# lkp411/cDLRM

Hardware: AMD Instinct MI355X
Metric: training samples/sec, Criteo-Terabyte-shape synthetic (cached data-parallel DLRM step; look-ahead refills that fall into the timed region included: see config.refills_in_timed_region) (higher is better)
Workload: dtype f32

## Files before the change

cdlrm_amd/csrc/dense.hip:

```cpp
#include "gemm_wide.h"
#include "gemm_bf16.h"

#define SK_KMAX 32
__global__ void __launch_bounds__(256) k_linear_smallk(const float* __restrict__ X, int64_t ld_x, const float* __restrict__ W,
                                                       const float* __restrict__ bias, float* __restrict__ Y, int64_t ld_y,
                                                       int64_t M, int N, int K, int act) {
    __shared__ float Xs[32][SK_KMAX + 1];
    __shared__ __attribute__((aligned(16))) float Wt[SK_KMAX][128 + 4];
    const int64_t m0 = (int64_t)blockIdx.y * 32;
    const int n0 = blockIdx.x * 128;
    for (int e = threadIdx.x; e < 32 * K; e += 256) {
        const int r = e / K, k = e % K;
        Xs[r][k] = X[min(m0 + r, M - 1) * ld_x + k];
    }
    for (int e = threadIdx.x; e < 128 * K; e += 256) {
        const int n = e / K, k = e % K;
        Wt[k][n] = W[(int64_t)min(n0 + n, N - 1) * K + k];
    }
    __syncthreads();
    const int cg = threadIdx.x & 31, rg = threadIdx.x >> 5;
    float acc[4][4];
#pragma unroll
    for (int i = 0; i < 4; ++i)
#pragma unroll
// ... 851 lines not shown
        const int off = itself ? 1 : 0;
#if IA_ABL == 3
        if (acc00[0] + acc10[1] + acc11[2] == 1.2345f) out[0] = 1.f;
#else
        for (int c = lane; c < D; c += 64) out[c] = Ts[c];
#pragma unroll
        for (int r = 0; r < 4; ++r) {
            const int i0 = 4 * g4 + r, i1 = 16 + 4 * g4 + r;
            if (i0 < F && l16 < i0 + off) out[D + pair_base(i0, itself) + l16] = acc00[r];
            if (i1 < F) out[D + pair_base(i1, itself) + l16] = acc10[r];
            if (i1 < F && 16 + l16 < i1 + off) out[D + pair_base(i1, itself) + 16 + l16] = acc11[r];
        }
#endif
        __builtin_amdgcn_sched_barrier(0);
        IA_STAMP_AT(3)
    };
    for (; b < B; b += nw) one(b);
}

struct IaGather {
    const TableDesc* tab;
    const v4f* weight;
    const int32_t* slots;
    int64_t n;
    int64_t ldx4;
    const uint8_t* once;
    int64_t ld_once;
    float lr;
};

template <int D4, int NS, bool G, bool DB = false>
__global__ void __launch_bounds__(256) k_interact_fwd_s(const float* __restrict__ feat, IaGather ga, int64_t B, int F,
                                                        int itself, float* __restrict__ R, int64_t ld_r) {
    constexpr int D = 4 * D4, CS = D4 / NS, DS = 4 * CS, PITCH = DS + 4, NR = CS / 2;
    constexpr int TSW = ia_fwd_s_slices(D4, NS, DB);
    static_assert(32 * PITCH == ia_slab_slice(D4, NS), "the slice the kernel walks is the slice the launch is sized for");
    static_assert(!DB || (NS % 2 == 0 && DS / 16 >= 1), "double buffering alternates two slices over an even number of slabs");
    extern __shared__ __attribute__((aligned(16))) float smem[];
    const int lane = threadIdx.x & 63, wave = threadIdx.x >> 6;
    float* Ts = smem + wave * ia_fwd_s_floats(D4, NS, DB);
    float* Os = Ts + TSW;
    const int64_t nw = (int64_t)gridDim.x * 4;
    int64_t b = (int64_t)blockIdx.x * 4 + wave;
    if (b >= B) return;
    const int l16 = lane & 15, g4 = lane >> 4;
    const int off = itself ? 1 : 0;
    int soff[NR], doff[NR];
    int srow[G ? NR : 1];
    const v4f* wbase[G ? NR : 1];
#pragma unroll
    for (int i = 0; i < NR; ++i) {
        const int e = lane + 64 * i, row = e / CS, c = e % CS;
        soff[i] = G ? c : min(row, F - 1) * D4 + c;
        doff[i] = row * PITCH + 4 * c;
        if constexpr (G) {
            const int t = max(min(row, F - 1) - 1, 0);
            srow[i] = t * (int)ga.n;
            wbase[i] = ga.weight + (ga.tab[t].row_base * D4 + c);
        }
    }
    v4f nxt[NS][NR];
    const v4f* pn[G ? NR : 1];
    int32_t sl[G ? NR : 1];
    auto load_slots = [&](int64_t bb) __attribute__((always_inline)) {
#pragma unroll
        for (int i = 0; i < NR; ++i) sl[i] = ga.slots[srow[i] + bb];
    };
    auto make_ptrs = [&](int64_t bb) __attribute__((always_inline)) {
#pragma unroll
        for (int i = 0; i < NR; ++i) {
            const v4f* p = wbase[i] + (int64_t)sl[i] * D4;
            if (i == 0 && lane < CS) p = reinterpret_cast<const v4f*>(feat) + bb * ga.ldx4 + soff[i];
            pn[i] = p;
        }
    };
    auto prefetch = [&](int s, int64_t bb) __attribute__((always_inline)) {
        if constexpr (G) {
#pragma unroll
            for (int i = 0; i < NR; ++i) nxt[s][i] = pn[i][s * CS];
        } else {
            const v4f* src = reinterpret_cast<const v4f*>(feat) + bb * (int64_t)F * D4 + s * CS;
#pragma unroll
            for (int i = 0; i < NR; ++i) nxt[s][i] = src[soff[i]];
        }
    };
    if constexpr (G) {
        load_slots(b);
        make_ptrs(b);
    }
#pragma unroll
    for (int s = 0; s < NS; ++s) prefetch(s, b);
    if constexpr (G) load_slots(min(b + nw, B - 1));
    if constexpr (DB) {
        float* const T0 = Ts;
        float* const T1 = Ts + 32 * PITCH;
        constexpr int NG = DS / 16;
#pragma unroll
        for (int i = 0; i < NR; ++i) *reinterpret_cast<v4f*>(T0 + doff[i]) = nxt[0][i];
        const int toff = l16 * PITCH + 4 * g4;
        float4 fa0 = *reinterpret_cast<const float4*>(T0 + toff);
        float4 fa1 = *reinterpret_cast<const float4*>(T0 + toff + 16 * PITCH);
        auto one_db = [&](int64_t b) __attribute__((always_inline)) {
            const int64_t bn = min(b + nw, B - 1);
            if constexpr (G) {
                make_ptrs(bn);
                load_slots(min(bn + nw, B - 1));
            }
            prefetch(0, bn);
            if (lane < CS) *reinterpret_cast<v4f*>(Os + 4 * lane) = *reinterpret_cast<const v4f*>(T0 + 4 * lane);
            v4f acc00 = {0.f, 0.f, 0.f, 0.f}, acc10 = acc00, acc11 = acc00;
            auto mf = [&](int j, const float4& a0, const float4& a1) __attribute__((always_inline)) {
                const int c = j / 3, w = j % 3;
                const float x0 = c == 0 ? a0.x : c == 1 ? a0.y : c == 2 ? a0.z : a0.w;
                const float x1 = c == 0 ? a1.x : c == 1 ? a1.y : c == 2 ? a1.z : a1.w;
                if (w == 0) acc00 = __builtin_amdgcn_mfma_f32_16x16x4f32(x0, x0, acc00, 0, 0, 0);
                else if (w == 1) acc10 = __builtin_amdgcn_mfma_f32_16x16x4f32(x1, x0, acc10, 0, 0, 0);
                else acc11 = __builtin_amdgcn_mfma_f32_16x16x4f32(x1, x1, acc11, 0, 0, 0);
            };
#pragma unroll
            for (int s = 0; s < NS; ++s) {
                const float* cur = (s & 1) ? T1 : T0;
                float* oth = (s & 1) ? T0 : T1;
#pragma unroll
                for (int g = 0; g < NG; ++g) {
                    const float4 a0 = fa0, a1 = fa1;
                    const float* np_ = (g + 1 < NG) ? cur + toff + 16 * (g + 1) : oth + toff;
#pragma unroll
                    for (int j = 0; j < 12; ++j) {
                        mf(j, a0, a1);
                        const int k = g * 12 + j;
                        if (k >= 0 && k < NR) {
                            const int sn = s + 1 < NS ? s + 1 : 0;
                            *reinterpret_cast<v4f*>(oth + doff[k]) = nxt[sn][k];
                        }
                        if (k == NR && s + 1 < NS && lane < CS) *reinterpret_cast<v4f*>(Os + (s + 1) * DS + 4 * lane) = nxt[s + 1][0];
                        if (k == NR + 1 && s + 1 < NS) prefetch(s + 1, bn);
                        if (j == (NG == 1 ? NR + 2 : 0) && g == NG - 1) {
                            fa0 = *reinterpret_cast<const float4*>(np_);
                            fa1 = *reinterpret_cast<const float4*>(np_ + 16 * PITCH);
                        }
                        if (j == 0 && g + 1 < NG) {
                            fa0 = *reinterpret_cast<const float4*>(np_);
                            fa1 = *reinterpret_cast<const float4*>(np_ + 16 * PITCH);
                        }
                        __builtin_amdgcn_sched_barrier(0);
                    }
                }
            }
            float* out = R + b * ld_r;
#pragma unroll
            for (int r = 0; r < 4; ++r) {
                const int i0 = 4 * g4 + r, i1 = 16 + 4 * g4 + r;
                if (i0 < F && l16 < i0 + off) Os[D + pair_base(i0, itself) + l16] = acc00[r];
                if (i1 < F) Os[D + pair_base(i1, itself) + l16] = acc10[r];
                if (i1 < F && 16 + l16 < i1 + off) Os[D + pair_base(i1, itself) + 16 + l16] = acc11[r];
            }
            const int width = D + pair_base(F, itself);
            if (lane < 4) Os[width + lane] = 0.f;
            const int W4 = (width + 3) >> 2;
            constexpr int NST = (D4 + 132 + 63) / 64;
#pragma unroll
            for (int k = 0; k < NST; ++k) {
                const int e = min(64 * k + lane, W4 - 1);
                *reinterpret_cast<v4f*>(out + 4 * e) = *reinterpret_cast<const v4f*>(Os + 4 * e);
            }
            __builtin_amdgcn_sched_barrier(0);
        };
        one_db(b);
        for (b += nw; b < B; b += nw) one_db(b);
        return;
    }
    auto one = [&](int64_t b) __attribute__((always_inline)) {
        const int64_t bn = min(b + nw, B - 1);
        if constexpr (G) {
            make_ptrs(bn);
            load_slots(min(bn + nw, B - 1));
        }
        v4f acc00 = {0.f, 0.f, 0.f, 0.f}, acc10 = acc00, acc11 = acc00;
        const float* tp = Ts + l16 * PITCH + 4 * g4;
#pragma unroll
        for (int s = 0; s < NS; ++s) {
#pragma unroll
            for (int i = 0; i < NR; ++i) *reinterpret_cast<v4f*>(Ts + doff[i]) = nxt[s][i];
            if (lane < CS) *reinterpret_cast<v4f*>(Os + s * DS + 4 * lane) = nxt[s][0];
            prefetch(s, bn);
            __builtin_amdgcn_sched_barrier(0);
#pragma unroll 2
            for (int g = 0; g < DS / 16; ++g) {
                const float4 a0 = *reinterpret_cast<const float4*>(tp + 16 * g);
                const float4 a1 = *reinterpret_cast<const float4*>(tp + 16 * PITCH + 16 * g);
                acc00 = __builtin_amdgcn_mfma_f32_16x16x4f32(a0.x, a0.x, acc00, 0, 0, 0);
                acc10 = __builtin_amdgcn_mfma_f32_16x16x4f32(a1.x, a0.x, acc10, 0, 0, 0);
                acc11 = __builtin_amdgcn_mfma_f32_16x16x4f32(a1.x, a1.x, acc11, 0, 0, 0);
                acc00 = __builtin_amdgcn_mfma_f32_16x16x4f32(a0.y, a0.y, acc00, 0, 0, 0);
                acc10 = __builtin_amdgcn_mfma_f32_16x16x4f32(a1.y, a0.y, acc10, 0, 0, 0);
                acc11 = __builtin_amdgcn_mfma_f32_16x16x4f32(a1.y, a1.y, acc11, 0, 0, 0);
                acc00 = __builtin_amdgcn_mfma_f32_16x16x4f32(a0.z, a0.z, acc00, 0, 0, 0);
                acc10 = __builtin_amdgcn_mfma_f32_16x16x4f32(a1.z, a0.z, acc10, 0, 0, 0);
                acc11 = __builtin_amdgcn_mfma_f32_16x16x4f32(a1.z, a1.z, acc11, 0, 0, 0);
                acc00 = __builtin_amdgcn_mfma_f32_16x16x4f32(a0.w, a0.w, acc00, 0, 0, 0);
                acc10 = __builtin_amdgcn_mfma_f32_16x16x4f32(a1.w, a0.w, acc10, 0, 0, 0);
                acc11 = __builtin_amdgcn_mfma_f32_16x16x4f32(a1.w, a1.w, acc11, 0, 0, 0);
            }
            __builtin_amdgcn_sched_barrier(0);
        }
        float* out = R + b * ld_r;
#pragma unroll
        for (int r = 0; r < 4; ++r) {
            const int i0 = 4 * g4 + r, i1 = 16 + 4 * g4 + r;
            if (i0 < F && l16 < i0 + off) Os[D + pair_base(i0, itself) + l16] = acc00[r];
            if (i1 < F) Os[D + pair_base(i1, itself) + l16] = acc10[r];
            if (i1 < F && 16 + l16 < i1 + off) Os[D + pair_base(i1, itself) + 16 + l16] = acc11[r];
        }
        const int width = D + pair_base(F, itself);
        if (lane < 4) Os[width + lane] = 0.f;
        const int W4 = (width + 3) >> 2;
        constexpr int NST = (D4 + 132 + 63) / 64;
#pragma unroll
        for (int k = 0; k < NST; ++k) {
            const int e = min(64 * k + lane, W4 - 1);
            *reinterpret_cast<v4f*>(out + 4 * e) = *reinterpret_cast<const v4f*>(Os + 4 * e);
        }
        __builtin_amdgcn_sched_barrier(0);
    };
    one(b);
    for (b += nw; b < B; b += nw) one(b);
}

template <int D4>
__global__ void __launch_bounds__(256) k_interact_bwd_p(const float* __restrict__ feat, const float* __restrict__ dR,
                                                        int64_t ld_r, int64_t B, int F, int itself, int x_act,
                                                        float* __restrict__ dfeat) {
    constexpr int D = 4 * D4, PITCH = D + 4;
    constexpr int GMAX = ia_grad_row(D4);
    constexpr int NG = (GMAX / 4 + 63) / 64;
    static_assert(32 * PITCH == ia_row_tile(D4), "the tile the kernel walks is the tile the launch is sized for");
    extern __shared__ __attribute__((aligned(16))) float smem[];
    const int lane = threadIdx.x & 63, wave = threadIdx.x >> 6;
    const int lr = lane & 31, lk = lane >> 5;
    float* Ts = smem + wave * ia_bwd_p_floats(D4);
    float* Gs = Ts + 32 * PITCH;
    for (int e = lane; e < 32 * PITCH; e += 64) Ts[e] = 0.f;
    const int FD4 = F * D4;
    const int off = itself ? 1 : 0;
    const int npairs = pair_base(F, itself);
    const int G4 = (D + npairs + 3) / 4;
    const int64_t nw = (int64_t)gridDim.x * 4;
    int64_t b = (int64_t)blockIdx.x * 4 + wave;
    if (b >= B) return;
    v4f nxt[D4 / 2], gn[NG];
    interact_prefetch<D4>(feat, b, FD4, lane, nxt);
#pragma unroll
    for (int i = 0; i < NG; ++i) gn[i] = reinterpret_cast<const v4f*>(dR + b * ld_r)[min(lane + 64 * i, G4 - 1)];
    auto one = [&](int64_t b) __attribute__((always_inline)) {
        interact_stage<D4>(Ts, FD4, lane, nxt);
#pragma unroll
        for (int i = 0; i < NG; ++i) *reinterpret_cast<v4f*>(Gs + 4 * min(lane + 64 * i, GMAX / 4 - 1)) = gn[i];
        const int64_t bn = min(b + nw, B - 1);
        interact_prefetch<D4>(feat, bn, FD4, lane, nxt);
#pragma unroll
        for (int i = 0; i < NG; ++i) gn[i] = reinterpret_cast<const v4f*>(dR + bn * ld_r)[min(lane + 64 * i, G4 - 1)];
        __builtin_amdgcn_sched_barrier(0);
        float sreg[16];
#pragma unroll
        for (int m = 0; m < 16; ++m) {
            const int j = lk + 2 * m;
            float v = 0.f;
            if (lr < F && j < F) {
                if (j < lr + off) v += Gs[D + pair_base(lr, itself) + j];
                if (lr < j + off) v += Gs[D + pair_base(j, itself) + lr];
            }
            sreg[m] = v;
        }
        float* out = dfeat + b * F * D;
        for (int n0 = 0; n0 < D; n0 += 32) {
            f32x16 acc;
#pragma unroll
            for (int r = 0; r < 16; ++r) acc[r] = 0.f;
            const float* tp = Ts + lk * PITCH + n0 + lr;
#pragma unroll
            for (int m = 0; m < 16; ++m) acc = __builtin_amdgcn_mfma_f32_32x32x2f32(sreg[m], tp[2 * m * PITCH], acc, 0, 0, 0);
            const int col = n0 + lr;
#pragma unroll
            for (int r = 0; r < 16; ++r) {
                const int i = (r & 3) + 8 * (r >> 2) + 4 * lk;
                if (i < F) {
                    float v = acc[r];
                    if (i == 0) {
                        v += Gs[col];
                        const float y = Ts[col];
                        if (x_act == 1) v = y > 0.f ? v : 0.f;
                        else if (x_act == 2) v = v * ((1.0f - y) * y);
                    }
                    out[i * D + col] = v;
                }
            }
        }
        __builtin_amdgcn_sched_barrier(0);
    };
    for (; b < B; b += nw) one(b);
}

template <int D4, int NS, bool G, bool ONCE = false>
__global__ void __launch_bounds__(256, (G && D4 <= 32) ? 2 : 1) k_interact_bwd_s(const float* __restrict__ feat, IaGather ga,
                                                        const float* __restrict__ dR, int64_t ld_r, int64_t B, int F,
                                                        int itself, int x_act, float* __restrict__ dfeat) {
    constexpr int D = 4 * D4, CS = D4 / NS, DS = 4 * CS, PITCH = DS + 4, NR = CS / 2;
    constexpr int GMAX = ia_grad_row(D4);
    constexpr int NG = (GMAX / 4 + 63) / 64;
    static_assert(DS % 32 == 0, "a slab is a whole number of 32-column MFMA blocks");
    static_assert(32 * PITCH == ia_slab_slice(D4, NS), "the slice the kernel walks is the slice the launch is sized for");
    extern __shared__ __attribute__((aligned(16))) float smem[];
    const int lane = threadIdx.x & 63, wave = threadIdx.x >> 6;
    const int lr = lane & 31, lk = lane >> 5;
    float* Ts = smem + wave * ia_bwd_s_floats(D4, NS);
    float* Gs = Ts + 32 * PITCH;
    float* Os = Gs + D;
    const int off = itself ? 1 : 0;
    const int npairs = pair_base(F, itself);
    const int G4 = (D + npairs + 3) / 4;
    const int64_t nw = (int64_t)gridDim.x * 4;
    int64_t b = (int64_t)blockIdx.x * 4 + wave;
    if (b >= B) return;
    int soff[NR], doff[NR];
    int srow[G ? NR : 1];
    int orow[ONCE ? NR : 1];
    const v4f* wbase[G ? NR : 1];
#pragma unroll
    for (int i = 0; i < NR; ++i) {
        const int e = lane + 64 * i, row = e / CS, c = e % CS;
        soff[i] = G ? c : min(row, F - 1) * D4 + c;
        doff[i] = row * PITCH + 4 * c;
        if constexpr (G) {
            const int t = max(min(row, F - 1) - 1, 0);
            srow[i] = t * (int)ga.n;
            if constexpr (ONCE) orow[i] = t * (int)ga.ld_once;
            wbase[i] = ga.weight + (ga.tab[t].row_base * D4 + c);
        }
    }
    static_assert(!ONCE || (G && CS == 8 && DS == 32), "the output store's lane -> (row, word) map is the staging map");
    v4f nxt[NS][NR], gn[NG];
    const v4f* pn[G ? NR : 1];
    int32_t sl[G ? NR : 1];
    const v4f* pc[ONCE ? NR : 1];
    uint8_t fl[ONCE ? NR : 1], fn[ONCE ? NR : 1], fc[ONCE ? NR : 1];
    auto load_slots = [&](int64_t bb) __attribute__((always_inline)) {
#pragma unroll
        for (int i = 0; i < NR; ++i) {
            sl[i] = ga.slots[srow[i] + bb];
            if constexpr (ONCE) fl[i] = ga.once[orow[i] + bb];
        }
    };
    auto make_ptrs = [&](int64_t bb) __attribute__((always_inline)) {
#pragma unroll
        for (int i = 0; i < NR; ++i) {
            const v4f* p = wbase[i] + (int64_t)sl[i] * D4;
            if constexpr (ONCE) fn[i] = fl[i];
            if (i == 0 && lane < CS) {
                p = reinterpret_cast<const v4f*>(feat) + bb * ga.ldx4 + soff[i];
                if constexpr (ONCE) fn[i] = 0;
            }
            pn[i] = p;
        }
    };
    auto prefetch = [&](int s, int64_t bb) __attribute__((always_inline)) {
        if constexpr (G) {
#pragma unroll
            for (int i = 0; i < NR; ++i) nxt[s][i] = pn[i][s * CS];
        } else {
            const v4f* src = reinterpret_cast<const v4f*>(feat) + bb * (int64_t)F * D4 + s * CS;
#pragma unroll
            for (int i = 0; i < NR; ++i) nxt[s][i] = src[soff[i]];
        }
    };
    if constexpr (G) {
        load_slots(b);
        make_ptrs(b);
    }
#pragma unroll
    for (int i = 0; i < NG; ++i) gn[i] = reinterpret_cast<const v4f*>(dR + b * ld_r)[min(lane + 64 * i, G4 - 1)];
#pragma unroll
    for (int s = 0; s < NS; ++s) prefetch(s, b);
    if constexpr (G) load_slots(min(b + nw, B - 1));
    auto one = [&](int64_t b) __attribute__((always_inline)) {
        const int64_t bn = min(b + nw, B - 1);
        if constexpr (G) {
            if constexpr (ONCE) {
#pragma unroll
                for (int i = 0; i < NR; ++i) { pc[i] = pn[i]; fc[i] = fn[i]; }
            }
            make_ptrs(bn);
            load_slots(min(bn + nw, B - 1));
        }
#pragma unroll
        for (int i = 0; i < NG; ++i) *reinterpret_cast<v4f*>(Gs + 4 * min(lane + 64 * i, GMAX / 4 - 1)) = gn[i];
#pragma unroll
        for (int i = 0; i < NG; ++i) gn[i] = reinterpret_cast<const v4f*>(dR + bn * ld_r)[min(lane + 64 * i, G4 - 1)];
        __builtin_amdgcn_sched_barrier(0);
        float sreg[16];
#pragma unroll
        for (int m = 0; m < 16; ++m) {
            const int j = lk + 2 * m;
            float v = 0.f;
            if (lr < F && j < F) {
                if (j < lr + off) v += Gs[D + pair_base(lr, itself) + j];
                if (lr < j + off) v += Gs[D + pair_base(j, itself) + lr];
            }
            sreg[m] = v;
        }
        float* out = dfeat + b * F * D;
#pragma unroll
        for (int s = 0; s < NS; ++s) {
#pragma unroll
            for (int i = 0; i < NR; ++i) *reinterpret_cast<v4f*>(Ts + doff[i]) = nxt[s][i];
            prefetch(s, bn);
            __builtin_amdgcn_sched_barrier(0);
#pragma unroll
            for (int nl = 0; nl < DS; nl += 32) {
                const int n0 = s * DS + nl;
                f32x16 acc;
#pragma unroll
                for (int r = 0; r < 16; ++r) acc[r] = 0.f;
                const float* tp = Ts + lk * PITCH + nl + lr;
#pragma unroll
                for (int m = 0; m < 16; ++m) acc = __builtin_amdgcn_mfma_f32_32x32x2f32(sreg[m], tp[2 * m * PITCH], acc, 0, 0, 0);
                {
                    float v = acc[0] + Gs[n0 + lr];
                    const float y = Ts[nl + lr];
                    if (x_act == 1) v = y > 0.f ? v : 0.f;
                    else if (x_act == 2) v = v * ((1.0f - y) * y);
                    acc[0] = lk == 0 ? v : acc[0];
                }
#pragma unroll
                for (int h = 0; h < 2; ++h) {
#pragma unroll
                    for (int rr = 0; rr < 8; ++rr)
                        Os[((rr & 3) + 8 * (rr >> 2) + 4 * lk) * 32 + lr] = acc[8 * h + rr];
                    const int nvalid = min(F - 16 * h, 16) * 8;
#pragma unroll
                    for (int k = 0; k < 2; ++k) {
                        const int idx = min(64 * k + lane, nvalid - 1);
                        const int row = idx >> 3, c4 = idx & 7;
                        const v4f gv = *reinterpret_cast<const v4f*>(Os + row * 32 + 4 * c4);
                        if constexpr (ONCE) {
                            if (64 * k + lane < nvalid && fc[2 * h + k]) {
                                v4f w = *reinterpret_cast<const v4f*>(Ts + (16 * h + row) * PITCH + nl + 4 * c4);
                                v4f a = {0.f, 0.f, 0.f, 0.f};
                                a += gv;
                                w.x = fmaf(-ga.lr, a.x, w.x); w.y = fmaf(-ga.lr, a.y, w.y);
                                w.z = fmaf(-ga.lr, a.z, w.z); w.w = fmaf(-ga.lr, a.w, w.w);
                                *const_cast<v4f*>(pc[2 * h + k] + s * CS) = w;
                                continue;
                            }
                        }
                        *reinterpret_cast<v4f*>(out + (16 * h + row) * D + n0 + 4 * c4) = gv;
                    }
                }
            }
            __builtin_amdgcn_sched_barrier(0);
        }
    };
    one(b);
    for (b += nw; b < B; b += nw) one(b);
}

enum { IA_FWD = CDLRM_IA_OP_FWD, IA_BWD = CDLRM_IA_OP_BWD, IA_GATHER_FWD = CDLRM_IA_OP_GATHER_FWD,
       IA_GATHER_BWD = CDLRM_IA_OP_GATHER_BWD, IA_GATHER_BWD_SGD = CDLRM_IA_OP_GATHER_BWD_SGD };

struct IaPlan {
    int family;
    int d4, ns;
    int64_t grid;
    size_t lds;
};

constexpr bool ia_gather_fwd_db(int d4) { return d4 > 8; }

static IaPlan interact_plan(int op, int64_t B, int F, int D, int itself, int64_t ld_r, bool aligned_r, bool aligned_dfeat) {
    IaPlan p{};
    const int npairs = itself ? F * (F + 1) / 2 : F * (F - 1) / 2, width = D + npairs;
    const bool piped = D == 32 || D == 64 || D == 128 || D == 256;
    const bool gather = op >= IA_GATHER_FWD;
    if (gather && !(piped && F > 16 && F <= 32)) return p;
    const bool vec = gather || (ld_r % 4 == 0 && aligned_r && ld_r >= ((width + 3) & ~3));
    const int d4 = D / 4, ns = d4 / 8;
    int floats;
    int64_t cap;
    p.d4 = d4;
    if (op == IA_GATHER_FWD) {
        const bool db = ia_gather_fwd_db(d4);
        p.family = db ? CDLRM_IA_SLAB_DB : CDLRM_IA_SLAB;
        p.ns = ns;
        floats = ia_fwd_s_floats(d4, ns, db);
        cap = 256 * (g_cdlrm_debug[4] > 0 ? g_cdlrm_debug[4] : 1);
    } else if (gather) {
        p.family = CDLRM_IA_SLAB;
        p.ns = ns;
        floats = ia_bwd_s_floats(d4, ns);
        cap = 256 * (g_cdlrm_debug[5] > 0 ? g_cdlrm_debug[5] : (D == 256 ? 1 : 2));
    } else if (op == IA_FWD && piped && vec) {
        p.family = CDLRM_IA_SLAB;
        p.ns = ns;
        floats = ia_fwd_s_floats(d4, ns, false);
        cap = 256;
    } else if (op == IA_FWD && piped) {
        p.family = CDLRM_IA_ROW;
        floats = ia_fwd_p_floats(d4);
        cap = 512;
    } else if (op == IA_FWD) {
        p.family = CDLRM_IA_GENERIC;
        floats = ia_generic_tile(D);
        cap = 2048;
    } else if (piped && vec && F > 16 && aligned_dfeat) {
        p.family = CDLRM_IA_SLAB;
        p.ns = ns;
        floats = ia_bwd_s_floats(d4, ns);
        cap = D == 256 ? 256 : 512;
    } else if (piped && D != 256 && vec) {
        p.family = CDLRM_IA_ROW;
        floats = ia_bwd_p_floats(d4);
        cap = 512;
    } else {
        p.family = CDLRM_IA_GENERIC;
        floats = ia_generic_bwd_floats(D, npairs);
        cap = 2048;
    }
    p.grid = cdiv(B, 4) < cap ? cdiv(B, 4) : cap;
    p.lds = (size_t)4 * floats * sizeof(float);
    return p;
}

template <typename Fn>
static int ia_with_d4(int d4, Fn&& fn) {
    switch (d4) {
        case 8: return fn(std::integral_constant<int, 8>{});
        case 16: return fn(std::integral_constant<int, 16>{});
        case 32: return fn(std::integral_constant<int, 32>{});
        case 64: return fn(std::integral_constant<int, 64>{});
    }
    cdlrm_set_error("interaction: no pipelined kernel at D = %d", 4 * d4);
    return CDLRM_EINVAL;
}

template <auto Kernel, typename... Args>
static int ia_launch(const IaPlan& p, void* stream, bool carry, Args... args) {
    const int rc = cdlrm_grant_dynamic_lds<Kernel>(p.lds);
    if (rc) return rc;
    const dim3 grid((unsigned)p.grid), block(256);
    if (carry) CDLRM_LAUNCH_EV(Kernel, grid, block, p.lds, (hipStream_t)stream, args...);
    else hipLaunchKernelGGL(Kernel, grid, block, p.lds, (hipStream_t)stream, args...);
    CDLRM_LAUNCH_CHECK();
    return 0;
}

extern "C" int cdlrm_interact_fwd(const float* feat, int64_t B, int32_t F, int32_t D, int32_t itself, float* R,
                                  int64_t ld_r, void* stream) {
    CDLRM_REQUIRE(feat && R && F >= 1 && F <= 32 && D >= 4 && D % 4 == 0 && D <= 512, "unsupported shape (F<=32, D%4==0)");
    CDLRM_REQUIRE(aligned16(feat) && ld_r >= D + (itself ? F * (F + 1) / 2 : F * (F - 1) / 2), "alignment / ld_r");
    if (B == 0) return 0;
    const IaPlan p = interact_plan(IA_FWD, B, F, D, itself, ld_r, aligned16(R), false);
    if (p.family == CDLRM_IA_SLAB)
        return ia_with_d4(p.d4, [&](auto d4) {
            constexpr int D4 = decltype(d4)::value;
            return ia_launch<k_interact_fwd_s<D4, D4 / 8, false>>(p, stream, false, feat, IaGather{}, B, F, itself, R, ld_r);
        });
    if (p.family == CDLRM_IA_ROW)
        return ia_with_d4(p.d4, [&](auto d4) {
            return ia_launch<k_interact_fwd_p<decltype(d4)::value>>(p, stream, false, feat, B, F, itself, R, ld_r);
        });
    return ia_launch<k_interact_fwd>(p, stream, false, feat, B, F, D, itself, R, ld_r);
}

extern "C" int cdlrm_interact_bwd(const float* feat, const float* dR, int64_t ld_r, int64_t B, int32_t F, int32_t D,
                                  int32_t itself, int32_t x_act, float* dfeat, void* stream) {
    CdlrmStopScope stop_scope;
    CDLRM_REQUIRE(feat && dR && dfeat && F >= 1 && F <= 32 && D >= 4 && D % 4 == 0 && D <= 512, "unsupported shape");
    CDLRM_REQUIRE(aligned16(feat), "alignment");
    if (B == 0) return 0;
    const IaPlan p = interact_plan(IA_BWD, B, F, D, itself, ld_r, aligned16(dR), aligned16(dfeat));
    if (p.family == CDLRM_IA_SLAB)
        return ia_with_d4(p.d4, [&](auto d4) {
            constexpr int D4 = decltype(d4)::value;
            return ia_launch<k_interact_bwd_s<D4, D4 / 8, false>>(p, stream, true, feat, IaGather{}, dR, ld_r, B, F, itself, x_act,
                                                                  dfeat);
        });
    if (p.family == CDLRM_IA_ROW)
        return ia_with_d4(p.d4, [&](auto d4) {
            constexpr int D4 = decltype(d4)::value;
            if constexpr (D4 <= 32)
                return ia_launch<k_interact_bwd_p<D4>>(p, stream, true, feat, dR, ld_r, B, F, itself, x_act, dfeat);
            else
                return (int)CDLRM_EINVAL;
        });
    CDLRM_REQUIRE(p.lds <= 160 * 1024, "LDS budget");
    return ia_launch<k_interact_bwd>(p, stream, false, feat, dR, ld_r, B, F, D, itself, x_act, dfeat);
}

extern "C" int cdlrm_interact_route(int32_t op, int64_t B, int32_t F, int32_t D, int32_t itself, int64_t ld_r,
                                    int32_t aligned, struct cdlrm_interact_route* out) {
    CDLRM_REQUIRE(out && op >= IA_FWD && op <= IA_GATHER_BWD_SGD && B >= 0, "bad argument");
    CDLRM_REQUIRE(F >= 1 && F <= 32 && D >= 4 && D % 4 == 0 && D <= 512, "unsupported shape (F<=32, D%4==0)");
    const int width = D + (itself ? F * (F + 1) / 2 : F * (F - 1) / 2);
    const IaPlan p = interact_plan(op, B, F, D, itself, ld_r, aligned & 1, aligned & 2);
    if (op == IA_FWD) CDLRM_REQUIRE(ld_r >= width, "alignment / ld_r");
    if (op == IA_BWD && p.family == CDLRM_IA_GENERIC) CDLRM_REQUIRE(p.lds <= 160 * 1024, "LDS budget");
    if (op >= IA_GATHER_FWD) {
        CDLRM_REQUIRE(p.family, "unsupported shape (D in 32/64/128/256, 16 < T + 1 <= 32)");
        CDLRM_REQUIRE(ld_r % 4 == 0 && (aligned & 1) && ld_r >= ((width + 3) & ~3) && (op == IA_GATHER_FWD || (aligned & 2)),
                      "whole-float4 output / gradient rows");
    }
    out->family = p.family; out->d4 = p.d4; out->ns = p.ns; out->reserved = 0;
    out->grid = p.grid; out->lds_bytes = (int64_t)p.lds;
    return 0;
}

extern "C" int cdlrm_gather_interact_supported(cdlrm_ctx* ctx) {
    return ctx && interact_plan(IA_GATHER_FWD, 1, ctx->T + 1, ctx->D, 0, 0, true, true).family ? 1 : 0;
}

extern "C" int cdlrm_gather_interact_fwd(cdlrm_ctx* ctx, const int32_t* slots, int64_t n, const float* x, int64_t ld_x,
                                         int64_t B, int32_t itself, float* R, int64_t ld_r, void* stream) {
    CdlrmStopScope stop_scope;
    CDLRM_CLEAR_STALE();
    CDLRM_REQUIRE(ctx && slots && x && R, "null argument");
    CDLRM_REQUIRE(ctx->weight, "cdlrm_ctx_bind_cache first");
    const int D = ctx->D, F = ctx->T + 1;
    const IaPlan p = interact_plan(IA_GATHER_FWD, B, F, D, itself, ld_r, aligned16(R), false);
    CDLRM_REQUIRE(p.family, "unsupported shape (D in 32/64/128/256, 16 < T + 1 <= 32): gather + interaction as two calls");
    const int width = D + (itself ? F * (F + 1) / 2 : F * (F - 1) / 2);
    CDLRM_REQUIRE(n >= B && (int64_t)ctx->T * n < INT32_MAX && aligned16(x) && ld_x % 4 == 0 && ld_x >= D,
                  "slot pitch / dense-feature rows");
    CDLRM_REQUIRE(ld_r % 4 == 0 && aligned16(R) && ld_r >= ((width + 3) & ~3), "whole-float4 output rows");
    if (B == 0) return 0;
    hipEvent_t ev0 = (hipEvent_t)ctx->ev_start, ev1 = (hipEvent_t)ctx->ev_stop;
    ctx->ev_start = ctx->ev_stop = nullptr;
    hipEvent_t se = cdlrm_take_stop_event((hipStream_t)stream);
    if (!ev1 && se) { ev1 = se; se = nullptr; }
    IaGather ga{ctx->d_tab, reinterpret_cast<const v4f*>(ctx->weight), slots, n, ld_x / 4};
    const int rc = ia_with_d4(p.d4, [&](auto d4) {
        constexpr int D4 = decltype(d4)::value;
        constexpr auto kernel = k_interact_fwd_s<D4, D4 / 8, true, ia_gather_fwd_db(D4)>;
        const int rc = cdlrm_grant_dynamic_lds<kernel>(p.lds);
        if (rc) return rc;
        hipExtLaunchKernelGGL(kernel, dim3((unsigned)p.grid), dim3(256), p.lds, (hipStream_t)stream, ev0, ev1, 0, x, ga, B, F,
                              itself, R, ld_r);
        return 0;
    });
    if (rc) return rc;
    if (se) CDLRM_HIP_CHECK(hipEventRecord(se, (hipStream_t)stream));
    CDLRM_LAUNCH_CHECK();
    return 0;
}

static int cdlrm_gather_interact_bwd_core(cdlrm_ctx* ctx, const int32_t* slots, int64_t n, const float* x, int64_t ld_x,
                               const float* dR, int64_t ld_r, int64_t B, int32_t itself, int32_t x_act,
                               float* dfeat, const uint8_t* once, int64_t ld_once, float lr, void* stream) {
    CdlrmStopScope stop_scope;
    CDLRM_REQUIRE(ctx && slots && x && dR && dfeat, "null argument");
    CDLRM_REQUIRE(ctx->weight, "cdlrm_ctx_bind_cache first");
    const int D = ctx->D, F = ctx->T + 1;
    const IaPlan p = interact_plan(once ? IA_GATHER_BWD_SGD : IA_GATHER_BWD, B, F, D, itself, ld_r, aligned16(dR), aligned16(dfeat));
    CDLRM_REQUIRE(p.family, "unsupported shape (D in 32/64/128/256, 16 < T + 1 <= 32): cdlrm_interact_bwd on a gathered block");
    const int npairs = itself ? F * (F + 1) / 2 : F * (F - 1) / 2;
    CDLRM_REQUIRE(n >= B && (int64_t)ctx->T * n < INT32_MAX && aligned16(x) && ld_x % 4 == 0 && ld_x >= D,
                  "slot pitch / dense-feature rows");
    CDLRM_REQUIRE(ld_r % 4 == 0 && aligned16(dR) && ld_r >= ((D + npairs + 3) & ~3) && aligned16(dfeat), "whole-float4 gradient rows");
    if (B == 0) return 0;
    IaGather ga{ctx->d_tab, reinterpret_cast<const v4f*>(ctx->weight), slots, n, ld_x / 4, once, ld_once, lr};
    return ia_with_d4(p.d4, [&](auto d4) {
        constexpr int D4 = decltype(d4)::value;
        if (once)
            return ia_launch<k_interact_bwd_s<D4, D4 / 8, true, true>>(p, stream, true, x, ga, dR, ld_r, B, F, itself, x_act, dfeat);
        return ia_launch<k_interact_bwd_s<D4, D4 / 8, true, false>>(p, stream, true, x, ga, dR, ld_r, B, F, itself, x_act, dfeat);
    });
}

extern "C" int cdlrm_gather_interact_bwd(cdlrm_ctx* ctx, const int32_t* slots, int64_t n, const float* x, int64_t ld_x,
                                         const float* dR, int64_t ld_r, int64_t B, int32_t itself, int32_t x_act,
                                         float* dfeat, void* stream) {
    return cdlrm_gather_interact_bwd_core(ctx, slots, n, x, ld_x, dR, ld_r, B, itself, x_act, dfeat, nullptr, 0, 0.f, stream);
}

extern "C" int cdlrm_gather_interact_bwd_sgd(cdlrm_ctx* ctx, const int32_t* slots, int64_t n, const float* x, int64_t ld_x,
                                             const float* dR, int64_t ld_r, int64_t B, int32_t itself, int32_t x_act,
                                             float* dfeat, const uint8_t* once, int64_t ld_once, float lr, void* stream) {
    if (!(ctx && once && ld_once >= B && (int64_t)ctx->T * ld_once < INT32_MAX)) {
        CdlrmStopScope stop_scope;
        CDLRM_REQUIRE(ctx && once, "null argument");
        CDLRM_REQUIRE(ld_once >= B && (int64_t)ctx->T * ld_once < INT32_MAX, "flag pitch");
    }
    return cdlrm_gather_interact_bwd_core(ctx, slots, n, x, ld_x, dR, ld_r, B, itself, x_act, dfeat, once, ld_once, lr, stream);
}

__global__ void __launch_bounds__(256) k_bce_partial(const float* __restrict__ Z, const float* __restrict__ T, int64_t n,
                                                     float* __restrict__ part, float* __restrict__ dZ,
                                                     int sigmoid_bwd) {
    __shared__ float red[4];
    float s = 0.f;
    const float inv_n = 1.0f / (float)n;
    for (int64_t i = (int64_t)blockIdx.x * blockDim.x + threadIdx.x; i < n; i += (int64_t)gridDim.x * blockDim.x) {
        const float z = Z[i], t = T[i];
        const float l1 = fmaxf(logf(z), -100.f), l0 = fmaxf(log1pf(-z), -100.f);
        s += (t - 1.0f) * l0 - t * l1;
        if (dZ) {
            float d = (z - t) / fmaxf((1.0f - z) * z, 1e-12f) * inv_n;
            if (sigmoid_bwd) d = d * ((1.0f - z) * z);
            dZ[i] = d;
        }
    }
#pragma unroll
    for (int d = 32; d >= 1; d >>= 1) s += __shfl_down(s, d, 64);
    if ((threadIdx.x & 63) == 0) red[threadIdx.x >> 6] = s;
    __syncthreads();
    if (threadIdx.x == 0) part[blockIdx.x] = red[0] + red[1] + red[2] + red[3];
}

__global__ void __launch_bounds__(1024) k_bce_one(const float* __restrict__ Z, const float* __restrict__ T, int64_t n,
                                                  float* __restrict__ loss, float* __restrict__ dZ, int sigmoid_bwd) {
    __shared__ float red[16];
    float s = 0.f;
    const float inv_n = 1.0f / (float)n;
    for (int64_t i0 = threadIdx.x; i0 < n; i0 += 8 * 1024) {
        float z[8], t[8];
#pragma unroll
        for (int u = 0; u < 8; ++u) {
            const int64_t i = min(i0 + u * 1024, n - 1);
            z[u] = Z[i];
            t[u] = T[i];
        }
#pragma unroll
        for (int u = 0; u < 8; ++u) {
            const int64_t i = i0 + u * 1024;
            if (i < n) {
                const float l1 = fmaxf(logf(z[u]), -100.f), l0 = fmaxf(log1pf(-z[u]), -100.f);
                s += (t[u] - 1.0f) * l0 - t[u] * l1;
                if (dZ) {
                    float d = (z[u] - t[u]) / fmaxf((1.0f - z[u]) * z[u], 1e-12f) * inv_n;
                    if (sigmoid_bwd) d = d * ((1.0f - z[u]) * z[u]);
                    dZ[i] = d;
                }
            }
        }
    }
#pragma unroll
    for (int d = 32; d >= 1; d >>= 1) s += __shfl_down(s, d, 64);
    if ((threadIdx.x & 63) == 0) red[threadIdx.x >> 6] = s;
    __syncthreads();
    if (threadIdx.x == 0) {
        float tot = 0.f;
#pragma unroll
        for (int w = 0; w < 16; ++w) tot += red[w];
        loss[0] = tot / (float)n;
    }
}

__global__ void __launch_bounds__(64) k_bce_final(const float* __restrict__ part, int nparts, int64_t n,
                                                  float* __restrict__ loss) {
    float s = 0.f;
// ... 377 lines not shown
```

Baseline: 15.20 million.

## Restructure interaction backward kernel: transposed MFMA output, shallow prefetch ring, direct stores

Swaps the MFMA operand order so each lane holds a row's output columns, which lets results be stored straight to global memory or folded into the embedding update without the LDS Os staging transpose. Replaces the full per-slab prefetch array with a shallower compile-time ring of depth PD and recomputes offsets on the fly, which cuts register use so occupancy can be raised to 3 waves per SIMD. The once-touched fold state is now tracked per output row. It also adds software-pipelined LDS operand loads for the MFMA chain and branch-free pair-gradient gathers. The risk is exposed global-load latency from the shallower prefetch, plus possible register spills under the tighter launch bound.

```diff
diff --git a/cdlrm_amd/csrc/dense.hip b/cdlrm_amd/csrc/dense.hip
--- a/cdlrm_amd/csrc/dense.hip
+++ b/cdlrm_amd/csrc/dense.hip
@@ -1177,7 +1177,7 @@
 }
 
 template <int D4, int NS, bool G, bool ONCE = false>
-__global__ void __launch_bounds__(256, (G && D4 <= 32) ? 2 : 1) k_interact_bwd_s(const float* __restrict__ feat, IaGather ga,
+__global__ void __launch_bounds__(256, (G && D4 <= 32) ? 3 : 1) k_interact_bwd_s(const float* __restrict__ feat, IaGather ga,
                                                         const float* __restrict__ dR, int64_t ld_r, int64_t B, int F,
                                                         int itself, int x_act, float* __restrict__ dfeat) {
     constexpr int D = 4 * D4, CS = D4 / NS, DS = 4 * CS, PITCH = DS + 4, NR = CS / 2;
@@ -1186,109 +1186,128 @@
     static_assert(DS % 32 == 0, "a slab is a whole number of 32-column MFMA blocks");
     static_assert(32 * PITCH == ia_slab_slice(D4, NS), "the slice the kernel walks is the slice the launch is sized for");
     extern __shared__ __attribute__((aligned(16))) float smem[];
-    const int lane = threadIdx.x & 63, wave = threadIdx.x >> 6;
+    const int lane = threadIdx.x & 63, wave = __builtin_amdgcn_readfirstlane(threadIdx.x >> 6);
     const int lr = lane & 31, lk = lane >> 5;
     float* Ts = smem + wave * ia_bwd_s_floats(D4, NS);
     float* Gs = Ts + 32 * PITCH;
-    float* Os = Gs + D;
     const int off = itself ? 1 : 0;
     const int npairs = pair_base(F, itself);
     const int G4 = (D + npairs + 3) / 4;
     const int64_t nw = (int64_t)gridDim.x * 4;
     int64_t b = (int64_t)blockIdx.x * 4 + wave;
     if (b >= B) return;
-    int soff[NR], doff[NR];
-    int srow[G ? NR : 1];
-    int orow[ONCE ? NR : 1];
+    constexpr int PD = D4 == 32 ? (ONCE ? 1 : 2) : NS;
+    static_assert(NS % PD == 0, "the ring place of a slab is a compile-time constant");
     const v4f* wbase[G ? NR : 1];
-#pragma unroll
-    for (int i = 0; i < NR; ++i) {
-        const int e = lane + 64 * i, row = e / CS, c = e % CS;
-        soff[i] = G ? c : min(row, F - 1) * D4 + c;
-        doff[i] = row * PITCH + 4 * c;
+    const int sc = G ? lane % CS : 0;
+    if constexpr (G) {
+#pragma unroll
+        for (int i = 0; i < NR; ++i) {
+            const int row = (lane + 64 * i) / CS;
+            const int t = max(min(row, F - 1) - 1, 0);
+            wbase[i] = ga.weight + (ga.tab[t].row_base * D4 + sc);
+        }
+    }
+    static_assert(!ONCE || (G && CS == 8 && DS == 32), "the fold reads its row's words of the one 32-column block of a slab");
+    v4f nxt[PD][NR], gn[NG];
+    int32_t slp[G ? NR : 1];
+    int32_t sl[G ? NR : 1];
+    const int ot = max(min(lr, F - 1) - 1, 0);
+    const bool orow_ok = lr >= 1 && lr < F;
+    int64_t obase = 0;
+    if constexpr (ONCE) obase = ga.tab[ot].row_base;
+    int32_t oc = 0, on = 0;
+    uint8_t of = 0, ofn = 0;
+    auto load_once = [&](int64_t bb) __attribute__((always_inline)) {
+        if constexpr (ONCE) {
+            on = ga.slots[ot * (int)ga.n + bb];
+            ofn = ga.once[ot * (int)ga.ld_once + bb];
+        }
+    };
+    auto load_slots = [&](int64_t bb) __attribute__((always_inline)) {
+        int lv = lane;
+        asm volatile("" : "+v"(lv));
+#pragma unroll
+        for (int i = 0; i < (G ? NR : 1); ++i)
+            sl[i] = ga.slots[max(min((lv + 64 * i) / CS, F - 1) - 1, 0) * (int)ga.n + bb];
+    };
+    auto next_sample = [&]() __attribute__((always_inline)) {
+#pragma unroll
+        for (int i = 0; i < (G ? NR : 1); ++i) slp[i] = sl[i];
+    };
+    auto prefetch = [&](int to, int s, int64_t bb) __attribute__((always_inline)) {
         if constexpr (G) {
-            const int t = max(min(row, F - 1) - 1, 0);
-            srow[i] = t * (int)ga.n;
-            if constexpr (ONCE) orow[i] = t * (int)ga.ld_once;
-            wbase[i] = ga.weight + (ga.tab[t].row_base * D4 + c);
-        }
-    }
-    static_assert(!ONCE || (G && CS == 8 && DS == 32), "the output store's lane -> (row, word) map is the staging map");
-    v4f nxt[NS][NR], gn[NG];
-    const v4f* pn[G ? NR : 1];
-    int32_t sl[G ? NR : 1];
-    const v4f* pc[ONCE ? NR : 1];
-    uint8_t fl[ONCE ? NR : 1], fn[ONCE ? NR : 1], fc[ONCE ? NR : 1];
-    auto load_slots = [&](int64_t bb) __attribute__((always_inline)) {
-#pragma unroll
-        for (int i = 0; i < NR; ++i) {
-            sl[i] = ga.slots[srow[i] + bb];
-            if constexpr (ONCE) fl[i] = ga.once[orow[i] + bb];
-        }
-    };
-    auto make_ptrs = [&](int64_t bb) __attribute__((always_inline)) {
-#pragma unroll
-        for (int i = 0; i < NR; ++i) {
-            const v4f* p = wbase[i] + (int64_t)sl[i] * D4;
-            if constexpr (ONCE) fn[i] = fl[i];
-            if (i == 0 && lane < CS) {
-                p = reinterpret_cast<const v4f*>(feat) + bb * ga.ldx4 + soff[i];
-                if constexpr (ONCE) fn[i] = 0;
-            }
-            pn[i] = p;
-        }
-    };
-    auto prefetch = [&](int s, int64_t bb) __attribute__((always_inline)) {
-        if constexpr (G) {
-#pragma unroll
-            for (int i = 0; i < NR; ++i) nxt[s][i] = pn[i][s * CS];
+#pragma unroll
+            for (int i = 0; i < NR; ++i) {
+                const v4f* p = wbase[i] + (int64_t)slp[i] * D4;
+                if (i == 0 && lane < CS) p = reinterpret_cast<const v4f*>(feat) + bb * ga.ldx4 + sc;
+                nxt[to][i] = p[s * CS];
+            }
         } else {
             const v4f* src = reinterpret_cast<const v4f*>(feat) + bb * (int64_t)F * D4 + s * CS;
 #pragma unroll
-            for (int i = 0; i < NR; ++i) nxt[s][i] = src[soff[i]];
+            for (int i = 0; i < NR; ++i) {
+                const int e = lane + 64 * i;
+                nxt[to][i] = src[min(e / CS, F - 1) * D4 + e % CS];
+            }
         }
     };
     if constexpr (G) {
         load_slots(b);
-        make_ptrs(b);
-    }
+        next_sample();
+    }
+    load_once(b);
 #pragma unroll
     for (int i = 0; i < NG; ++i) gn[i] = reinterpret_cast<const v4f*>(dR + b * ld_r)[min(lane + 64 * i, G4 - 1)];
 #pragma unroll
-    for (int s = 0; s < NS; ++s) prefetch(s, b);
+    for (int s = 0; s < PD; ++s) prefetch(s, s, b);
     if constexpr (G) load_slots(min(b + nw, B - 1));
     auto one = [&](int64_t b) __attribute__((always_inline)) {
         const int64_t bn = min(b + nw, B - 1);
-        if constexpr (G) {
-            if constexpr (ONCE) {
-#pragma unroll
-                for (int i = 0; i < NR; ++i) { pc[i] = pn[i]; fc[i] = fn[i]; }
-            }
-            make_ptrs(bn);
-            load_slots(min(bn + nw, B - 1));
+        if constexpr (ONCE) {
+            oc = on;
+            of = orow_ok ? ofn : (uint8_t)0;
+            load_once(bn);
         }
 #pragma unroll
         for (int i = 0; i < NG; ++i) *reinterpret_cast<v4f*>(Gs + 4 * min(lane + 64 * i, GMAX / 4 - 1)) = gn[i];
 #pragma unroll
         for (int i = 0; i < NG; ++i) gn[i] = reinterpret_cast<const v4f*>(dR + bn * ld_r)[min(lane + 64 * i, G4 - 1)];
         __builtin_amdgcn_sched_barrier(0);
+        int lrv = lr, lkv = lk;
+        asm volatile("" : "+v"(lrv), "+v"(lkv));
+        const int pbr = D + pair_base(lrv, itself);
         float sreg[16];
 #pragma unroll
         for (int m = 0; m < 16; ++m) {
-            const int j = lk + 2 * m;
+            const int j = lkv + 2 * m;
+            const bool in = lrv < F && j < F, lo = in && j < lrv + off, up = in && lrv < j + off;
+            const float glo = Gs[lo ? pbr + j : D], gup = Gs[up ? D + pair_base(j, itself) + lrv : D];
             float v = 0.f;
-            if (lr < F && j < F) {
-                if (j < lr + off) v += Gs[D + pair_base(lr, itself) + j];
-                if (lr < j + off) v += Gs[D + pair_base(j, itself) + lr];
-            }
+            v = lo ? v + glo : v;
+            v = up ? v + gup : v;
             sreg[m] = v;
-        }
-        float* out = dfeat + b * F * D;
+            if (m % 4 == 3) {
+                asm volatile("" : "+v"(sreg[m - 3]), "+v"(sreg[m - 2]), "+v"(sreg[m - 1]), "+v"(sreg[m]));
+                __builtin_amdgcn_sched_barrier(0);
+            }
+        }
+        float* out = dfeat + b * F * D + lr * D + 4 * lk;
 #pragma unroll
         for (int s = 0; s < NS; ++s) {
 #pragma unroll
-            for (int i = 0; i < NR; ++i) *reinterpret_cast<v4f*>(Ts + doff[i]) = nxt[s][i];
-            prefetch(s, bn);
+            for (int i = 0; i < NR; ++i) {
+                const int e = lane + 64 * i;
+                *reinterpret_cast<v4f*>(Ts + (e / CS) * PITCH + 4 * (e % CS)) = nxt[s % PD][i];
+            }
+            if constexpr (G) {
+                if (s == NS - PD) {
+                    next_sample();
+                    load_slots(min(bn + nw, B - 1));
+                }
+            }
+            if (s + PD < NS) prefetch(s % PD, s + PD, b);
+            else prefetch(s % PD, s + PD - NS, bn);
             __builtin_amdgcn_sched_barrier(0);
 #pragma unroll
             for (int nl = 0; nl < DS; nl += 32) {
@@ -1297,38 +1316,60 @@
 #pragma unroll
                 for (int r = 0; r < 16; ++r) acc[r] = 0.f;
                 const float* tp = Ts + lk * PITCH + nl + lr;
-#pragma unroll
-                for (int m = 0; m < 16; ++m) acc = __builtin_amdgcn_mfma_f32_32x32x2f32(sreg[m], tp[2 * m * PITCH], acc, 0, 0, 0);
-                {
-                    float v = acc[0] + Gs[n0 + lr];
-                    const float y = Ts[nl + lr];
-                    if (x_act == 1) v = y > 0.f ? v : 0.f;
-                    else if (x_act == 2) v = v * ((1.0f - y) * y);
-                    acc[0] = lk == 0 ? v : acc[0];
+                float af[2][4];
+#pragma unroll
+                for (int m = 0; m < 4; ++m) af[0][m] = tp[2 * m * PITCH];
+#pragma unroll
+                for (int g = 0; g < 4; ++g) {
+                    if (g < 3) {
+#pragma unroll
+                        for (int m = 0; m < 4; ++m) af[(g + 1) & 1][m] = tp[2 * (4 * g + 4 + m) * PITCH];
+                    }
+                    __builtin_amdgcn_sched_barrier(0);
+#pragma unroll
+                    for (int m = 0; m < 4; ++m)
+                        acc = __builtin_amdgcn_mfma_f32_32x32x2f32(af[g & 1][m], sreg[4 * g + m], acc, 0, 0, 0);
+                    __builtin_amdgcn_sched_barrier(0);
                 }
-#pragma unroll
-                for (int h = 0; h < 2; ++h) {
-#pragma unroll
-                    for (int rr = 0; rr < 8; ++rr)
-                        Os[((rr & 3) + 8 * (rr >> 2) + 4 * lk) * 32 + lr] = acc[8 * h + rr];
-                    const int nvalid = min(F - 16 * h, 16) * 8;
-#pragma unroll
-                    for (int k = 0; k < 2; ++k) {
-                        const int idx = min(64 * k + lane, nvalid - 1);
-                        const int row = idx >> 3, c4 = idx & 7;
-                        const v4f gv = *reinterpret_cast<const v4f*>(Os + row * 32 + 4 * c4);
-                        if constexpr (ONCE) {
-                            if (64 * k + lane < nvalid && fc[2 * h + k]) {
-                                v4f w = *reinterpret_cast<const v4f*>(Ts + (16 * h + row) * PITCH + nl + 4 * c4);
-                                v4f a = {0.f, 0.f, 0.f, 0.f};
-                                a += gv;
-                                w.x = fmaf(-ga.lr, a.x, w.x); w.y = fmaf(-ga.lr, a.y, w.y);
-                                w.z = fmaf(-ga.lr, a.z, w.z); w.w = fmaf(-ga.lr, a.w, w.w);
-                                *const_cast<v4f*>(pc[2 * h + k] + s * CS) = w;
-                                continue;
-                            }
+                if (lr == 0) {
+#pragma unroll
+                    for (int q = 0; q < 4; ++q) {
+                        const v4f gx = *reinterpret_cast<const v4f*>(Gs + n0 + 8 * q + 4 * lk);
+                        const v4f y4 = *reinterpret_cast<const v4f*>(Ts + nl + 8 * q + 4 * lk);
+#pragma unroll
+                        for (int t = 0; t < 4; ++t) acc[4 * q + t] = acc[4 * q + t] + gx[t];
+                        if (x_act == 1) {
+#pragma unroll
+                            for (int t = 0; t < 4; ++t) acc[4 * q + t] = y4[t] > 0.f ? acc[4 * q + t] : 0.f;
+                        } else if (x_act == 2) {
+#pragma unroll
+                            for (int t = 0; t < 4; ++t) acc[4 * q + t] = acc[4 * q + t] * ((1.0f - y4[t]) * y4[t]);
                         }
-                        *reinterpret_cast<v4f*>(out + (16 * h + row) * D + n0 + 4 * c4) = gv;
+                    }
+                }
+                bool fold = false;
+                if constexpr (ONCE) fold = of != 0;
+                if (fold) {
+                    if constexpr (ONCE) {
+                        v4f* wrow = const_cast<v4f*>(ga.weight) + ((obase + oc) * D4 + s * CS + lk);
+                        const float* ws = Ts + lr * PITCH + nl + 4 * lk;
+#pragma unroll
+                        for (int q = 0; q < 4; ++q) {
+                            v4f w = *reinterpret_cast<const v4f*>(ws + 8 * q);
+                            const v4f gv = {acc[4 * q], acc[4 * q + 1], acc[4 * q + 2], acc[4 * q + 3]};
+                            v4f a = {0.f, 0.f, 0.f, 0.f};
+                            a += gv;
+                            w.x = fmaf(-ga.lr, a.x, w.x); w.y = fmaf(-ga.lr, a.y, w.y);
+                            w.z = fmaf(-ga.lr, a.z, w.z); w.w = fmaf(-ga.lr, a.w, w.w);
+                            wrow[2 * q] = w;
+                            __builtin_amdgcn_sched_barrier(0);
+                        }
+                    }
+                } else if (lr < F) {
+#pragma unroll
+                    for (int q = 0; q < 4; ++q) {
+                        const v4f gv = {acc[4 * q], acc[4 * q + 1], acc[4 * q + 2], acc[4 * q + 3]};
+                        *reinterpret_cast<v4f*>(out + n0 + 8 * q) = gv;
                     }
                 }
             }
```

New measurement: 14.92 million. 1.9% lower.
